# vasil-pashov/sparse_matrix_math

Hardware: AMD Instinct MI355X
Metric: CSR SpMV GB/s (% HBM peak) + BiCGStab iters/sec, 10M rows, 1/2/4/8 GPU (higher is better)
Workload: dtype f32

## Files before the change

include/smm_hip.h:

```cpp
#ifndef SMM_HIP_H
#define SMM_HIP_H

#include <stddef.h>

#ifdef __cplusplus
extern "C" {
#endif

#define SMM_HIP_VERSION_MAJOR 0
#define SMM_HIP_VERSION_MINOR 1

#define SMM_HIP_OK 0
#define SMM_HIP_ERR_INVALID (-1)
#define SMM_HIP_ERR_HIP (-2)
#define SMM_HIP_ERR_NO_DEVICE (-3)
#define SMM_HIP_ERR_PRECOND (-4)
#define SMM_HIP_ERR_NOMEM (-5)
#define SMM_HIP_ERR_COMM (-6)

#define SMM_SOLVER_SUCCESS 0
#define SMM_SOLVER_DIVERGED 1
#define SMM_SOLVER_MAX_ITERATIONS_REACHED 2

#define SMM_OP_ASSIGN 0
// ... 23 lines not shown

typedef struct smm_hip_csr smm_hip_csr;
typedef struct smm_hip_precond smm_hip_precond;
typedef void* smm_hip_stream;

int smm_hip_init(int device);
int smm_hip_shutdown(void);
const char* smm_hip_last_error(void);
int smm_hip_uses_std_fma(void);
int smm_hip_device_info(char* name, size_t name_cap, int* cus, size_t* hbm_bytes);
int smm_hip_stream_synchronize(smm_hip_stream stream);

int smm_hip_debug_fail_next_alloc(size_t min_bytes);
int smm_hip_profile_enable(int on);
int smm_hip_profile_read(double* spmv_ms, long long* spmv_launches, int reset);
int smm_hip_profile_read_waits(double* exposed_ms, long long* pairs, int reset);

int smm_hip_csr_create_f32(int rows, int cols, const int* start, const int* positions, const float* values, smm_hip_csr** out);
int smm_hip_csr_create_f64(int rows, int cols, const int* start, const int* positions, const double* values, smm_hip_csr** out);
int smm_hip_csr_create_dev_f32(int rows, int cols, const int* d_start, const int* d_positions, const float* d_values, smm_hip_csr** out);
int smm_hip_csr_create_dev_f64(int rows, int cols, const int* d_start, const int* d_positions, const double* d_values, smm_hip_csr** out);
int smm_hip_csr_destroy(smm_hip_csr* m);
int smm_hip_csr_info(const smm_hip_csr* m, int* rows, int* cols, int* nnz, int* dtype, int* first_active_start);
int smm_hip_csr_set_kernel(smm_hip_csr* m, int family, int lanes_per_row);
int smm_hip_csr_get_kernel(const smm_hip_csr* m, int* family, int* lanes_per_row);
int smm_hip_csr_tile_info(const smm_hip_csr* m, int* tiles, int* tile_nnz_cap, int* tile_max_rows, int* tile_kernel);
int smm_hip_csr_pattern_info(const smm_hip_csr* m, int* encoding, int* offsets);
int smm_hip_csr_kernel_desc(const smm_hip_csr* m, char* name, int name_cap, long long* bytes_per_launch);
int smm_hip_set_march_min_rows(long long const_diagonals_rows, long long values_read_rows);
int smm_hip_set_cg_lazy_x_min_bytes(long long bytes);
int smm_hip_set_cg_fuse_p(int on);
int smm_hip_csr_pattern_allow_const(smm_hip_csr* m, int allow);
int smm_hip_csr_pattern_slots(smm_hip_csr* m, int mode);
int smm_hip_csr_autotune(smm_hip_csr* m);

#define SMM_UPDATE_SET 0
#define SMM_UPDATE_ADD 1
int smm_hip_csr_scale_f32(smm_hip_csr* m, float alpha, smm_hip_stream stream);
int smm_hip_csr_scale_f64(smm_hip_csr* m, double alpha, smm_hip_stream stream);
int smm_hip_csr_axpy_f32(smm_hip_csr* m, float alpha, const smm_hip_csr* other, smm_hip_stream stream);
int smm_hip_csr_axpy_f64(smm_hip_csr* m, double alpha, const smm_hip_csr* other, smm_hip_stream stream);
int smm_hip_csr_zero_f32(smm_hip_csr* m, smm_hip_stream stream);
int smm_hip_csr_zero_f64(smm_hip_csr* m, smm_hip_stream stream);
int smm_hip_csr_update_entries_f32(smm_hip_csr* m, int n, const int* rows, const int* cols, const float* values, int mode, unsigned char* found);
int smm_hip_csr_update_entries_f64(smm_hip_csr* m, int n, const int* rows, const int* cols, const double* values, int mode, unsigned char* found);
int smm_hip_csr_update_entries_dev_f32(smm_hip_csr* m, int n, const int* d_rows, const int* d_cols, const float* d_values, int mode, unsigned char* d_found,
                                       smm_hip_stream stream);
int smm_hip_csr_update_entries_dev_f64(smm_hip_csr* m, int n, const int* d_rows, const int* d_cols, const double* d_values, int mode, unsigned char* d_found,
                                       smm_hip_stream stream);
int smm_hip_csr_set_values_f32(smm_hip_csr* m, const float* values);
int smm_hip_csr_set_values_f64(smm_hip_csr* m, const double* values);
int smm_hip_csr_set_values_dev_f32(smm_hip_csr* m, const float* d_values, smm_hip_stream stream);
int smm_hip_csr_set_values_dev_f64(smm_hip_csr* m, const double* d_values, smm_hip_stream stream);
int smm_hip_csr_get_values_f32(const smm_hip_csr* m, float* values);
int smm_hip_csr_get_values_f64(const smm_hip_csr* m, double* values);
int smm_hip_csr_values_changed_f32(smm_hip_csr* m, smm_hip_stream stream);
int smm_hip_csr_values_changed_f64(smm_hip_csr* m, smm_hip_stream stream);
int smm_hip_csr_same_pattern(const smm_hip_csr* a, const smm_hip_csr* b, int* same);

int smm_hip_spmv_f32(const smm_hip_csr* m, int op, const float* lhs, const float* x, float* out);
int smm_hip_spmv_f64(const smm_hip_csr* m, int op, const double* lhs, const double* x, double* out);
int smm_hip_spmv_dev_f32(const smm_hip_csr* m, int op, const float* d_lhs, const float* d_x, float* d_out, smm_hip_stream stream);
int smm_hip_spmv_dev_f64(const smm_hip_csr* m, int op, const double* d_lhs, const double* d_x, double* d_out, smm_hip_stream stream);

int smm_hip_dot_f32(int n, const float* a, const float* b, float* result);
int smm_hip_dot_f64(int n, const double* a, const double* b, double* result);
// ... 177 lines not shown
```

sparse_matrix_math_amd/_lib.py:

```python
import ctypes
import os
from ctypes import POINTER, c_char_p, c_double, c_float, c_int, c_longlong, c_size_t, c_ulonglong, c_void_p

_HERE = os.path.dirname(os.path.abspath(__file__))

SMM_HIP_OK = 0
SMM_HIP_ERR_INVALID = -1
SMM_HIP_ERR_HIP = -2
SMM_HIP_ERR_NO_DEVICE = -3
SMM_HIP_ERR_PRECOND = -4
SMM_HIP_ERR_NOMEM = -5
SMM_HIP_ERR_COMM = -6


class SmmHipError(RuntimeError):
    def __init__(self, code, message):
        super().__init__(f"libsmm_hip error {code}: {message}")
        self.code = code


def library_path(fma=False):
    if os.environ.get("SMM_HIP_LIBRARY"):
        return os.environ["SMM_HIP_LIBRARY"]
    name = "libsmm_hip_fma.so" if fma else "libsmm_hip.so"
# ... 46 lines not shown
    "smm_hip_csr_update_entries_dev": (c_int, [_P, c_int, _P, _P, _P, c_int, _P, _P]),
    "smm_hip_csr_set_values": (c_int, [_P, _P]),
    "smm_hip_csr_set_values_dev": (c_int, [_P, _P, _P]),
    "smm_hip_csr_get_values": (c_int, [_P, _P]),
    "smm_hip_csr_values_changed": (c_int, [_P, _P]),
}



_PLAIN = {
    "smm_hip_init": (c_int, [c_int]),
    "smm_hip_shutdown": (c_int, []),
    "smm_hip_last_error": (c_char_p, []),
    "smm_hip_uses_std_fma": (c_int, []),
    "smm_hip_device_info": (c_int, [c_char_p, c_size_t, POINTER(c_int), POINTER(c_size_t)]),
    "smm_hip_stream_synchronize": (c_int, [_P]),
    "smm_hip_debug_fail_next_alloc": (c_int, [c_size_t]),
    "smm_hip_profile_enable": (c_int, [c_int]),
    "smm_hip_profile_read": (c_int, [POINTER(c_double), POINTER(c_longlong), c_int]),
    "smm_hip_profile_read_waits": (c_int, [POINTER(c_double), POINTER(c_longlong), c_int]),
    "smm_hip_csr_destroy": (c_int, [_P]),
    "smm_hip_csr_info": (c_int, [_P, POINTER(c_int), POINTER(c_int), POINTER(c_int), POINTER(c_int), POINTER(c_int)]),
    "smm_hip_csr_set_kernel": (c_int, [_P, c_int, c_int]),
    "smm_hip_csr_get_kernel": (c_int, [_P, POINTER(c_int), POINTER(c_int)]),
    "smm_hip_csr_autotune": (c_int, [_P]),
    "smm_hip_csr_tile_info": (c_int, [_P, POINTER(c_int), POINTER(c_int), POINTER(c_int), POINTER(c_int)]),
    "smm_hip_csr_pattern_info": (c_int, [_P, POINTER(c_int), POINTER(c_int)]),
    "smm_hip_csr_kernel_desc": (c_int, [_P, c_char_p, c_int, POINTER(c_longlong)]),
    "smm_hip_set_march_min_rows": (c_int, [c_longlong, c_longlong]),
    "smm_hip_set_cg_lazy_x_min_bytes": (c_int, [c_longlong]),
    "smm_hip_set_cg_fuse_p": (c_int, [c_int]),
    "smm_hip_csr_pattern_allow_const": (c_int, [_P, c_int]),
    "smm_hip_csr_pattern_slots": (c_int, [_P, c_int]),
    "smm_hip_csr_same_pattern": (c_int, [_P, _P, POINTER(c_int)]),
    "smm_hip_precond_create": (c_int, [_P, c_int, POINTER(_P)]),
    "smm_hip_precond_create_block": (c_int, [_P, c_int, c_int, POINTER(_P)]),
    "smm_hip_precond_create_block_capped": (c_int, [_P, c_int, c_int, c_int, POINTER(_P)]),
    "smm_hip_precond_block_level_cap": (c_int, [_P, POINTER(c_int)]),
    "smm_hip_precond_create_block_ex": (c_int, [_P, c_int, c_int, c_int, c_int, POINTER(_P)]),
    "smm_hip_precond_block_rows": (c_int, [_P, _P, c_size_t, _P]),
    "smm_hip_precond_block_record_bytes": (c_int, [_P, POINTER(c_int), POINTER(c_int), POINTER(c_int)]),
    "smm_hip_precond_block_count": (c_int, [_P, POINTER(c_int)]),
    "smm_hip_precond_block_bounds": (c_int, [_P, _P, c_size_t]),
    "smm_hip_precond_destroy": (c_int, [_P]),
    "smm_hip_precond_set_sweep": (c_int, [_P, c_int]),
    "smm_hip_precond_take_error": (c_int, [_P, _P]),
    "smm_hip_precond_info": (c_int, [_P, POINTER(c_int), POINTER(c_int), POINTER(c_int)]),
    "smm_hip_gen_poisson2d_nnz": (c_longlong, [c_int, c_int]),
    "smm_hip_gen_stencil3d_nnz": (c_longlong, [c_int, c_int, c_int]),
    "smm_hip_gen_banded_nnz": (c_longlong, [c_int, c_int, c_ulonglong, c_int]),
    "smm_hip_gen_banded_row_start": (c_longlong, [c_int, c_int, c_ulonglong, c_int, c_int]),
    "smm_hip_partials_count": (c_int, []),
    "smm_hip_finish_len": (c_int, []),
    "smm_hip_finish_totals_offset": (c_int, []),
    "smm_hip_cg_resident": (c_int, [c_int]),
    "smm_hip_bicgstab_resident": (c_int, [c_int]),
    "smm_hip_bicgstab_ws_destroy": (c_int, [_P]),
    "smm_hip_cg_ws_status": (c_int, [_P, _P, POINTER(c_int)]),
    "smm_hip_bicgstab_ws_bind": (c_int, [_P, _P, _P, _P]),
    "smm_hip_bicgstab_ws_pointers": (c_int, [_P, POINTER(_P), POINTER(_P), POINTER(_P), POINTER(_P), POINTER(_P), POINTER(_P)]),
    "smm_hip_comm_unique_id": (c_int, [_P]),
    "smm_hip_comm_create_rccl": (c_int, [c_int, c_int, _P, POINTER(_P)]),
    "smm_hip_comm_create_host": (c_int, [c_int, c_int, HOST_ALLREDUCE_FN, HOST_SENDRECV_FN, _P, POINTER(_P)]),
    "smm_hip_comm_create_self": (c_int, [POINTER(_P)]),
    "smm_hip_comm_destroy": (c_int, [_P]),
    "smm_hip_comm_info": (c_int, [_P, POINTER(c_int), POINTER(c_int), POINTER(c_int)]),
# ... 86 lines not shown
```

sparse_matrix_math_amd/csrc/smm_internal.h:

```cpp
#pragma once
#include <hip/hip_runtime.h>

#include <cstddef>
#include <cstdint>
#include <cstdio>
#include <atomic>
#include <chrono>
#include <cstdlib>
#include <cstring>
#include <mutex>
#include <string>
#include <type_traits>
#include <vector>

#include "../../include/smm_hip.h"

namespace smm {

void setError(const char* fmt, ...);
int hipFail(hipError_t e, const char* what, const char* file, int line);

#define SMM_HIP_TRY(expr)                                             \
	do {                                                              \
		hipError_t _e = (expr);                                       \
// ... 179 lines not shown
constexpr int SPMV_ADD_DIV = 0x1000;
constexpr int SPMV_OP_ADD_DIV = 4;
constexpr int SPMV_HALF_TILES = 0x2000;
constexpr int SPMV_NO_FULL_ROWS = 0x4000;
constexpr int PARTS_TOTALS = 2 * NPART;
constexpr int PARTS_TICKETS = 16;
constexpr int PARTS_LEN = 2 * NPART + 2 + 2 * (PARTS_TICKETS + 1);
template <typename T>
__host__ __device__ inline unsigned* partsTicket(T* partials) { return reinterpret_cast<unsigned*>(partials + PARTS_TOTALS + 2); }
inline int spmvOutFlags(const smm_hip_csr* m, size_t elemBytes) {
	static const int forced = [] {
		const char* env = getenv("SMM_HIP_NT_OUT");
		return env ? atoi(env) : -1;
	}();
	if (forced >= 0) return forced ? SPMV_NT_OUT : 0;
	return static_cast<double>(m->rows) * static_cast<double>(elemBytes) >= 64.0 * 1024 * 1024 ? SPMV_NT_OUT : 0;
}

int buildRowBlocks(smm_hip_csr* m, int capNnz, int maxRows, hipStream_t s);
int buildTileTable(const smm_hip_csr* m, int capNnz, int maxRows, hipStream_t s, int** blocks, int* nBlocks, int* chunkTiles);
int cutRows(const int* d_start, int rows, long long nnz, int capNnz, int maxRows, hipStream_t s, int2** tiles, int* nTiles, int tilesPerChunk = 0);
int ensureCsrReady(const smm_hip_csr* m, hipStream_t s, bool streamKnown);
int ensurePattern(smm_hip_csr* m, hipStream_t s = nullptr, bool streamKnown = false, bool quiet = false, bool masksOnly = false);
int adoptPatternForSolver(const smm_hip_csr* m, int plannedIterations, hipStream_t s);
void adoptPatternQuietly(const smm_hip_csr* m, hipStream_t s);
int patternLanesFor(const smm_hip_csr* m);
const char* patternKernelDesc(const smm_hip_csr* m, int lanes, long long* bytes);
void planMarch(smm_hip_csr* m);
int refreshResEll(smm_hip_csr* a, hipStream_t s);
bool ensurePatternSlots(smm_hip_csr* m, int lanes, hipStream_t s);
bool patternSlotsChosen(const smm_hip_csr* m, int lanes);
long long patternSlotsBytes(const smm_hip_csr* m);
int refreshPatternSlots(smm_hip_csr* m, hipStream_t s);
int marchBuildMasks32(smm_hip_csr* m, hipStream_t s);
template <typename K>
inline int occupancyCached(std::atomic<long long>& slot, K kernel, int tpb, size_t lds, int fallback) {
	const long long seen = slot.load(std::memory_order_acquire);
	if (seen != 0 && static_cast<size_t>(seen >> 8) == lds) return static_cast<int>(seen & 0xFF);
	int n = 0;
	if (hipOccupancyMaxActiveBlocksPerMultiprocessor(&n, kernel, tpb, lds) != hipSuccess || n < 1) {
		(void)hipGetLastError();
		n = fallback;
	}
	n = n > 255 ? 255 : n;
	slot.store((static_cast<long long>(lds) << 8) | n, std::memory_order_release);
	return n;
}
template <typename K>
inline bool ensureDynamicLds(std::atomic<int>& granted, K kernel, size_t lds) {
	if (lds <= 64 * 1024) return true;
	int have = granted.load(std::memory_order_acquire);
	while (static_cast<size_t>(have) < lds) {
		if (hipFuncSetAttribute(reinterpret_cast<const void*>(kernel), hipFuncAttributeMaxDynamicSharedMemorySize, static_cast<int>(lds)) != hipSuccess) {
			(void)hipGetLastError();
			return false;
		}
		if (granted.compare_exchange_weak(have, static_cast<int>(lds), std::memory_order_acq_rel)) break;
	}
	return true;
}
inline int forcedWgsPerCU() {
	static const int forced = [] {
		const char* env = getenv("SMM_HIP_STREAM_WGS_PER_CU");
		return env ? (atoi(env) > 1 ? atoi(env) : 1) : 0;
	}();
	return forced;
}

bool cgHalfTiles(const smm_hip_csr* m, size_t elemBytes);
long long cgLazyMinBytes();
bool updateNT(long long n, size_t elemBytes, int vectors);
bool masksMarchApplies(const smm_hip_csr* m);
bool constMarchApplies(const smm_hip_csr* m);
template <typename T>
bool launchPatMasksMarch(const smm_hip_csr* m, int op, const T* lhs, const T* divisor, const T* x, T* out, int dotMode, const T* w1, T* partials,
                         const int* doneFlag, hipStream_t s);
template <typename T>
bool launchPatConstMarch(const smm_hip_csr* m, int op, const T* lhs, const T* divisor, const T* x, T* out, int dotMode, const T* w1, T* partials,
                         const int* doneFlag, hipStream_t s);
template <typename T>
void launchPatSlots(const smm_hip_csr* m, int lanes, int op, const T* lhs, const T* divisor, const T* x, T* out, int dotMode, const T* w1, T* partials,
                    const int* doneFlag, hipStream_t s);
template <typename T>
int launchSpmvPattern(const smm_hip_csr* m, int lanes, int op, const T* lhs, const T* divisor, const T* x, T* out, int dotMode, const T* w1, T* partials,
                      const int* doneFlag, hipStream_t s);
void chooseSpmvConfig(smm_hip_csr* m);
template <typename T>
int launchSpmvSplit(const smm_hip_csr* aLoc, const smm_hip_csr* aRem, int op, const T* lhs, const T* divisor, const T* own, const T* ext, T* out, int dotMode,
                    const T* w1, T* partials, const int* doneFlag, int extraFlags, const unsigned long long* landed, unsigned long long seq, unsigned long long* err,
                    long long ticks, hipStream_t s, const struct P2PSlotArgs* slots = nullptr, int sumsLdsMax = 16384, unsigned long long* waited = nullptr);
void launchSplitSignal(unsigned long long* landed, unsigned long long seq, hipStream_t s);
void preloadSplitUnit();
template <typename T>
struct CgFuseBook {
	const int* pad = nullptr;
	T* rrPing = nullptr;
	T* res = nullptr;
	int *iters = nullptr, *done = nullptr, *status = nullptr, *flushIter = nullptr;
};
template <typename T>
struct CgFuseArgs {
	const T* r;
	T* pNew;
	CgFuseBook<T> bk;
	const T* partsC;
	T eps;
	int par, iter;
	const T* totalsC = nullptr;
	int extraFlags = 0;
};
bool constMarchFusable(const smm_hip_csr* m, size_t elemBytes);
template <typename T>
bool launchConstMarchFusedP(const smm_hip_csr* m, const T* pOld, T* Ap, T* partials, const int* doneFlag, const CgFuseArgs<T>& f, hipStream_t s);

template <typename T>
// ... 100 lines not shown
```

sparse_matrix_math_amd/csrc/smm_spmv_pattern.hip:

```cpp
#include <algorithm>
#include <cmath>

#include <rocprim/device/device_radix_sort.hpp>

#include "smm_device.h"
#include "smm_internal.h"
#include "smm_pattern_dev.h"

namespace smm {

__global__ __launch_bounds__(TPB) void patBuildMasks(int rows, const int* __restrict__ meta, const int* __restrict__ offs, const int* __restrict__ start,
                                                     const int* __restrict__ positions, unsigned long long* __restrict__ masks,
                                                     int* __restrict__ flags, const void* __restrict__ values, int elemBytes,
                                                     const unsigned long long* __restrict__ cvalBits) {
	if (meta[1] != 0) return;
	const int k = meta[0];
	if (values != nullptr && k > 32) values = nullptr;
	int* mismatch = flags;
	__shared__ int sOff[MAXOFF];
	__shared__ unsigned long long sCval[MAXOFF];
	const bool checkConst = values != nullptr && flags[1] == 0;
	if (checkConst && threadIdx.x < k) sCval[threadIdx.x] = cvalBits[threadIdx.x];
	bool varies = false;
	__shared__ int sRow[TPB / WAVE][WAVE + 1];
// ... 1465 lines not shown
		return "spmvDictKernel";
	}
	if (L == 1 && m->pat_const && !m->pat_const_off) {
		static const bool marchOn = [] {
			const char* env = getenv("SMM_HIP_CONST_MARCH");
			return env ? atoi(env) != 0 : true;
		}();
		const bool march = marchOn && constMarchApplies(m);
		const bool bytesMasks = march && !m->march_clusters && m->d_pat_masks8 && m->pat_k - m->march_lo - m->march_hi == 5;
		*bytes = rows * (bytesMasks ? 1 : march ? 4 : 8) + vectors;
		return march ? (m->march_clusters ? "spmvPatternConstMarch3Kernel" : "spmvPatternConstMarchKernel") : "spmvPatternConstKernel";
	}
	*bytes = nnz * s + rows * 8 + startBytes + vectors;
	if (L == 1 && masksMarchApplies(m)) {
		static const bool masksMarchOn = [] {
			const char* env = getenv("SMM_HIP_MASKS_MARCH");
			return env ? atoi(env) != 0 : true;
		}();
		if (masksMarchOn) {
			*bytes = nnz * s + rows + (rows / 64 + 1) * 4 + vectors;
			return "spmvPatternMasksMarchKernel";
		}
	}
	if (L == 1) {
		static const int waveEnv = [] {
			const char* env = getenv("SMM_HIP_PATTERN_WAVE");
			return env ? atoi(env) : -1;
		}();
		if (waveEnv != 0 && m->pat_k <= 16) return "spmvPatternWaveKernel";
	}
	if ((L == 2 || L == 4) && patUseTile(L)) {
		if (patternSlotsChosen(m, L)) {
			*bytes = patternSlotsBytes(m);
			return "spmvPatternSlotsKernel";
		}
		return "spmvPatternTileKernel";
	}
	return "spmvPatternKernel";
}

static bool patNeedsTiles(const smm_hip_csr* m, int L) {
	if (L != 1 || m->pat_encoding != 0) return true;
	if (m->pat_const && !m->pat_const_off) return false;
	static const int waveEnv = [] {
		const char* env = getenv("SMM_HIP_PATTERN_WAVE");
		return env ? atoi(env) : -1;
	}();
	return !(waveEnv != 0 && m->pat_k <= 16);
}

static int buildPatternTiles(smm_hip_csr* m, int capNnz, int maxRows, hipStream_t s) {
	int* blocks = nullptr;
	int n = 0, chunk = 0;
	SMM_TRY(buildTileTable(m, capNnz, maxRows, s, &blocks, &n, &chunk));
	devFree(m->d_pat_rowblocks);
	m->d_pat_rowblocks = blocks;
	m->pat_n_rowblocks = n;
	m->pat_nnz_cap = capNnz;
	m->pat_max_rows = maxRows;
	m->pat_chunk_tiles = chunk;
	return SMM_HIP_OK;
}

template <typename T>
int launchSpmvPattern(const smm_hip_csr* m, int lanes, int op, const T* lhs, const T* divisor, const T* x, T* out, int dotMode, const T* w1, T* partials,
                      const int* doneFlag, hipStream_t s) {
	auto* mm = const_cast<smm_hip_csr*>(m);
// ... 52 lines not shown
```

sparse_matrix_math_amd/csrc/smm_spmv_slots.hip:

```cpp
#include <algorithm>

#include <rocprim/device/device_scan.hpp>

#include "smm_pattern_dev.h"

namespace smm {

constexpr int SLOT_WAVES = TPB / WAVE;

__global__ __launch_bounds__(TPB) void slotsCountKernel(int rows, int nWaves, const unsigned long long* __restrict__ masks, long long* __restrict__ counts,
                                                        int* __restrict__ uniformWaves) {
	const int lane = threadIdx.x & (WAVE - 1);
	int mine = 0;
	for (int w = (blockIdx.x * TPB + threadIdx.x) / WAVE; w < nWaves; w += gridDim.x * SLOT_WAVES) {
		const int row = w * WAVE + lane;
		const unsigned long long mm = row < rows ? masks[row] : ~0ULL;
		const unsigned long long lead = patUniform64(mm);
		const bool uniform = lead != 0ULL && __builtin_amdgcn_ballot_w64(!(row < rows && mm == lead)) == 0ULL;
		if (lane == 0) {
			counts[w] = uniform ? static_cast<long long>(__builtin_popcountll(lead)) * WAVE : 0;
			mine += uniform;
		}
	}
	if (lane == 0 && mine) atomicAdd(uniformWaves, mine);
}

__global__ __launch_bounds__(TPB) void slotsMarkKernel(int nWaves, const long long* __restrict__ counts, long long* __restrict__ base) {
	for (int w = blockIdx.x * TPB + threadIdx.x; w < nWaves; w += gridDim.x * TPB) {
		if (counts[w] == 0) base[w] = -1;
	}
}

template <typename T>
__global__ __launch_bounds__(TPB) void slotsFillKernel(int nWaves, const long long* __restrict__ base, const unsigned long long* __restrict__ masks,
                                                       const int* __restrict__ start, const T* __restrict__ values, T* __restrict__ slots) {
	const int lane = threadIdx.x & (WAVE - 1);
	for (int w = (blockIdx.x * TPB + threadIdx.x) / WAVE; w < nWaves; w += gridDim.x * SLOT_WAVES) {
		const long long b = base[w];
		if (b < 0) continue;
		const int row = w * WAVE + lane;
		const int len = __builtin_popcountll(masks[w * WAVE]);
// ... 57 lines not shown
				}
			}
			dot = part[0];
#pragma unroll
			for (int q = 1; q < L; ++q) dot += part[q];
		} else if (row < rows) {
			dot = patRowDirect<T, L>(start[row], start[row + 1], values, positions, x);
		}
		if (row < rows) {
			const T o = patApplyOp(op, lhs, divisor, row, dot);
			storeOut(out + row, o, ntOut);
			if (dotMode == 2) acc0 += o * o;
			if (dotMode) acc1 += o * w1[row];
		}
	}
	if (dotMode) {
		if (dotMode == 2) {
			const T s0 = blockSum256(acc0, red);
			if (t == 0) partials[blockIdx.x] = s0;
		}
		const T s1 = blockSum256(acc1, red);
		if (t == 0) partials[(dotMode == 2 ? NPART : 0) + blockIdx.x] = s1;
		for (int i = gridDim.x + blockIdx.x * TPB + t; i < NPART; i += gridDim.x * TPB) {
			partials[i] = T(0);
			if (dotMode == 2) partials[NPART + i] = T(0);
		}
		if (opFlags & SPMV_FINISH) lastBlockSums<T>(partials, NPART, dotMode == 2 ? 2 : 1, partials + PARTS_TOTALS, partsTicket(partials));
	}
}

static int slotsEnvMode() {
	static const int mode = [] {
		const char* env = getenv("SMM_HIP_PATTERN_SLOTS");
		return env ? (atoi(env) != 0 ? 1 : 0) : -1;
	}();
	return mode;
}

static int slotsMode(const smm_hip_csr* m) { return m->pat_slots_mode >= 0 ? m->pat_slots_mode : slotsEnvMode(); }

static bool slotsApplies(const smm_hip_csr* m, int lanes) {
	if (lanes != 2 && lanes != 4) return false;
	if (m->pat_encoding != 0 || (m->pat_const && !m->pat_const_off)) return false;
	static const bool fullRows = [] {
		const char* env = getenv("SMM_HIP_FULL_ROWS");
		const char* variant = getenv("SMM_HIP_PATTERN_VARIANT");
		return !(env && atoi(env) == 0) && !(variant && atoi(variant) == 0);
	}();
	return fullRows;
}

static bool slotsWanted(const smm_hip_csr* m, int lanes, bool* forced) {
	const int mode = slotsMode(m);
	*forced = mode == 1;
	if (mode == 0 || !slotsApplies(m, lanes)) return false;
	return mode == 1 || mode == 2 || !m->kernelForced;
}

static bool slotsUniformEnough(const smm_hip_csr* m) {
	return static_cast<long long>(m->pat_slots_uniform) * 100 >= static_cast<long long>(m->pat_slots_waves) * 99;
}

bool patternSlotsChosen(const smm_hip_csr* m, int lanes) {
	bool forced = false;
	if (!slotsWanted(m, lanes, &forced) || m->pat_slots_state != 1 || !m->d_pat_slots) return false;
	return forced || slotsUniformEnough(m);
}

template <typename T>
static int slotsFill(smm_hip_csr* m, hipStream_t s) {
	const int nWaves = m->pat_slots_waves;
	const int grid = std::max(1, std::min(4096, (nWaves + SLOT_WAVES - 1) / SLOT_WAVES));
	slotsFillKernel<T><<<grid, TPB, 0, s>>>(nWaves, m->d_pat_slot_base, m->d_pat_masks, m->d_start, static_cast<const T*>(m->d_values),
	                                         static_cast<T*>(m->d_pat_slots));
	SMM_HIP_TRY(hipGetLastError());
	return SMM_HIP_OK;
}

template <typename T>
static int slotsBuild(smm_hip_csr* m, bool forced, hipStream_t s) {
	SetupTrace trace("pattern: slots copy");
	const int nWaves = (m->rows + WAVE - 1) / WAVE;
	DevBuf<long long> counts, base;
	DevBuf<int> uniform;
	DevBuf<unsigned char> temp;
	SMM_TRY(counts.alloc(nWaves));
	SMM_TRY(base.alloc(static_cast<size_t>(nWaves) + 1));
	SMM_TRY(uniform.alloc(1));
	SMM_HIP_TRY(hipMemsetAsync(uniform.p, 0, sizeof(int), s));
	SMM_HIP_TRY(hipMemsetAsync(base.p, 0, sizeof(long long), s));
	const int grid = std::max(1, std::min(4096, (nWaves + SLOT_WAVES - 1) / SLOT_WAVES));
	slotsCountKernel<<<grid, TPB, 0, s>>>(m->rows, nWaves, m->d_pat_masks, counts.p, uniform.p);
	SMM_HIP_TRY(hipGetLastError());
	size_t tempBytes = 0;
	SMM_HIP_TRY(rocprim::inclusive_scan(nullptr, tempBytes, counts.p, base.p + 1, static_cast<size_t>(nWaves), rocprim::plus<long long>(), s));
	SMM_TRY(temp.alloc(tempBytes ? tempBytes : 1));
	SMM_HIP_TRY(rocprim::inclusive_scan(temp.p, tempBytes, counts.p, base.p + 1, static_cast<size_t>(nWaves), rocprim::plus<long long>(), s));
	slotsMarkKernel<<<std::max(1, std::min(4096, (nWaves + TPB - 1) / TPB)), TPB, 0, s>>>(nWaves, counts.p, base.p);
	SMM_HIP_TRY(hipGetLastError());
// ... 63 lines not shown
	const int g = (p + nb - 1) / nb;
	return g <= 8 ? 8 : g <= 13 ? 13 : 16;
}

template <typename T, int L, int G>
static void launchSlotsG(const smm_hip_csr* m, int op, const T* lhs, const T* divisor, const T* x, T* out, int dotMode, const T* w1, T* partials,
                         const int* doneFlag, hipStream_t s) {
	static std::atomic<long long> occ{0};
	const int perCU = occupancyCached(occ, spmvPatternSlotsKernel<T, L, G>, TPB, 0, 4);
	const int cus = (op & SPMV_LEAVE_ROOM) ? std::max(8, numCUs() - 8) : numCUs();
	const int nWaves = m->pat_slots_waves;
	const int grid = std::max(1, std::min(std::min((nWaves + SLOT_WAVES - 1) / SLOT_WAVES, cus * perCU), NPART));
	const int nGroups = std::min(8, grid);
	const int chunkWaves = (nWaves + nGroups - 1) / nGroups;
	spmvPatternSlotsKernel<T, L, G><<<grid, TPB, 0, s>>>(m->rows, nWaves, chunkWaves, m->d_pat_off, m->d_pat_slot_base, m->d_pat_masks,
	                                                    static_cast<const T*>(m->d_pat_slots), m->d_start, m->d_positions, static_cast<const T*>(m->d_values),
	                                                    (op & ~SPMV_LEAVE_ROOM) | spmvOutFlags(m, sizeof(T)), lhs, divisor, x, out, dotMode, w1, partials,
	                                                    doneFlag);
}

template <typename T, int L>
static void launchSlotsL(const smm_hip_csr* m, int op, const T* lhs, const T* divisor, const T* x, T* out, int dotMode, const T* w1, T* partials,
                         const int* doneFlag, hipStream_t s) {
	switch (slotsBatch(m, L)) {
	case 8: launchSlotsG<T, L, 8>(m, op, lhs, divisor, x, out, dotMode, w1, partials, doneFlag, s); break;
	case 13: launchSlotsG<T, L, 13>(m, op, lhs, divisor, x, out, dotMode, w1, partials, doneFlag, s); break;
	default: launchSlotsG<T, L, 16>(m, op, lhs, divisor, x, out, dotMode, w1, partials, doneFlag, s); break;
	}
}

template <typename T>
void launchPatSlots(const smm_hip_csr* m, int lanes, int op, const T* lhs, const T* divisor, const T* x, T* out, int dotMode, const T* w1, T* partials,
                    const int* doneFlag, hipStream_t s) {
	if (lanes == 2) {
		launchSlotsL<T, 2>(m, op, lhs, divisor, x, out, dotMode, w1, partials, doneFlag, s);
	} else {
		launchSlotsL<T, 4>(m, op, lhs, divisor, x, out, dotMode, w1, partials, doneFlag, s);
	}
}

template void launchPatSlots<float>(const smm_hip_csr*, int, int, const float*, const float*, const float*, float*, int, const float*, float*, const int*,
                                    hipStream_t);
template void launchPatSlots<double>(const smm_hip_csr*, int, int, const double*, const double*, const double*, double*, int, const double*, double*,
                                     const int*, hipStream_t);

}

extern "C" int smm_hip_csr_pattern_slots(smm_hip_csr* m, int mode) {
	if (!m || mode < -1 || mode > 2) {
		smm::setError("csr_pattern_slots: null matrix or a mode other than -1, 0, 1, 2");
		return SMM_HIP_ERR_INVALID;
	}
	std::lock_guard<std::mutex> lock(m->tileMutex);
	m->pat_slots_mode = mode;
	if (mode == 1 && m->pat_slots_state < 0) m->pat_slots_state = 0;
	return SMM_HIP_OK;
}
```

sparse_matrix_math_amd/host.py:

```python
import ctypes
import enum

import numpy as np

from . import _lib
from ._lib import check


class SolverStatus(enum.IntEnum):
    SUCCESS = 0
    DIVERGED = 1
    MAX_ITERATIONS_REACHED = 2


class SolverPreconditioner(enum.IntEnum):
    NONE = 0
    JACOBI = 1
    ILU0 = 2
    SYMMETRIC_GAUS_SEIDEL = 3
    IC0 = 4
    BLOCK_ILU0 = 5
    BLOCK_SGS = 6


# ... 48 lines not shown

def partials_count():
    return _lib.load().smm_hip_partials_count()


def finish_len():
    return _lib.load().smm_hip_finish_len()


def finish_totals_offset():
    return _lib.load().smm_hip_finish_totals_offset()


def uses_std_fma():
    return bool(_lib.load().smm_hip_uses_std_fma())


def synchronize(stream=None):
    check(_lib.load().smm_hip_stream_synchronize(_dptr(stream)))


def profile_enable(on=True):
    check(_lib.load().smm_hip_profile_enable(1 if on else 0))


def profile_read(reset=True):
    ms, n = ctypes.c_double(), ctypes.c_longlong()
    check(_lib.load().smm_hip_profile_read(ctypes.byref(ms), ctypes.byref(n), 1 if reset else 0))
    return ms.value, n.value


def set_march_min_rows(const_diagonals_rows=-1, values_read_rows=-1):
    check(_lib.load().smm_hip_set_march_min_rows(int(const_diagonals_rows), int(values_read_rows)))


def profile_read_waits(reset=True):
    ms, n = ctypes.c_double(), ctypes.c_longlong()
    check(_lib.load().smm_hip_profile_read_waits(ctypes.byref(ms), ctypes.byref(n), 1 if reset else 0))
    return ms.value, n.value


class Preconditioner:

    def __init__(self, matrix, kind, block_rows=None, level_cap=None, partition=None):
        self.matrix = matrix
        self.kind = SolverPreconditioner(kind)
        self._h = ctypes.c_void_p()
        if block_rows is None and level_cap is None and partition is None:
            check(_lib.load().smm_hip_precond_create(matrix._h, int(kind), ctypes.byref(self._h)))
        elif level_cap is None and partition is None:
            check(_lib.load().smm_hip_precond_create_block(matrix._h, int(kind), int(block_rows), ctypes.byref(self._h)))
        else:
            check(_lib.load().smm_hip_precond_create_block_ex(matrix._h, int(kind), int(block_rows or 0), -1 if level_cap is None else int(level_cap),
                                                               int(partition or 0), ctypes.byref(self._h)))

    def block_record_bytes(self):
        v = [ctypes.c_int() for _ in range(3)]
        check(_lib.load().smm_hip_precond_block_record_bytes(self._h, *[ctypes.byref(c) for c in v]))
        return tuple(c.value for c in v)

    def block_rows(self):
        n = self.matrix.rows
        order = np.zeros(n, dtype=np.int32)
        brick = (ctypes.c_int * 3)()
        check(_lib.load().smm_hip_precond_block_rows(self._h, order.ctypes.data_as(ctypes.c_void_p), n, ctypes.cast(brick, ctypes.c_void_p)))
        return order, tuple(brick)
# ... 363 lines not shown
```

Baseline: 893.5.

## Add row-sweep pattern SpMV kernel that keeps multiple wave-rows open for x reuse

Adds a new pattern-slots SpMV kernel in which each wave processes several consecutive 64-row groups at once. Waves are partitioned into per-XCD chunks so that x accesses across diagonals stay within a narrow sweeping window and hit in cache, instead of each diagonal front streaming x separately. A host heuristic compares the diagonal gaps against the swept block span to decide when to use it, for f32 only. This adds register pressure from R accumulators and more template instantiations, and the heuristic may pick it on matrices where it does not help.

```diff
diff --git a/include/smm_hip.h b/include/smm_hip.h
--- a/include/smm_hip.h
+++ b/include/smm_hip.h
@@ -79,6 +79,7 @@
 int smm_hip_set_cg_fuse_p(int on);
 int smm_hip_csr_pattern_allow_const(smm_hip_csr* m, int allow);
 int smm_hip_csr_pattern_slots(smm_hip_csr* m, int mode);
+int smm_hip_set_pattern_sweep_rows(int rows_open);
 int smm_hip_csr_autotune(smm_hip_csr* m);
 
 #define SMM_UPDATE_SET 0
diff --git a/sparse_matrix_math_amd/_lib.py b/sparse_matrix_math_amd/_lib.py
--- a/sparse_matrix_math_amd/_lib.py
+++ b/sparse_matrix_math_amd/_lib.py
@@ -102,6 +102,7 @@
     "smm_hip_set_cg_fuse_p": (c_int, [c_int]),
     "smm_hip_csr_pattern_allow_const": (c_int, [_P, c_int]),
     "smm_hip_csr_pattern_slots": (c_int, [_P, c_int]),
+    "smm_hip_set_pattern_sweep_rows": (c_int, [c_int]),
     "smm_hip_csr_same_pattern": (c_int, [_P, _P, POINTER(c_int)]),
     "smm_hip_precond_create": (c_int, [_P, c_int, POINTER(_P)]),
     "smm_hip_precond_create_block": (c_int, [_P, c_int, c_int, POINTER(_P)]),
diff --git a/sparse_matrix_math_amd/csrc/smm_internal.h b/sparse_matrix_math_amd/csrc/smm_internal.h
--- a/sparse_matrix_math_amd/csrc/smm_internal.h
+++ b/sparse_matrix_math_amd/csrc/smm_internal.h
@@ -235,6 +235,8 @@
 bool patternSlotsChosen(const smm_hip_csr* m, int lanes);
 long long patternSlotsBytes(const smm_hip_csr* m);
 int refreshPatternSlots(smm_hip_csr* m, hipStream_t s);
+int patternSweepRows(const smm_hip_csr* m, int lanes);
+int patternSweepGroupWaves(const smm_hip_csr* m, int lanes, int rowsOpen);
 int marchBuildMasks32(smm_hip_csr* m, hipStream_t s);
 template <typename K>
 inline int occupancyCached(std::atomic<long long>& slot, K kernel, int tpb, size_t lds, int fallback) {
@@ -284,6 +286,9 @@
 template <typename T>
 void launchPatSlots(const smm_hip_csr* m, int lanes, int op, const T* lhs, const T* divisor, const T* x, T* out, int dotMode, const T* w1, T* partials,
                     const int* doneFlag, hipStream_t s);
+template <typename T>
+void launchPatSweep(const smm_hip_csr* m, int lanes, int rowsOpen, int op, const T* lhs, const T* divisor, const T* x, T* out, int dotMode, const T* w1,
+                    T* partials, const int* doneFlag, hipStream_t s);
 template <typename T>
 int launchSpmvPattern(const smm_hip_csr* m, int lanes, int op, const T* lhs, const T* divisor, const T* x, T* out, int dotMode, const T* w1, T* partials,
                       const int* doneFlag, hipStream_t s);
diff --git a/sparse_matrix_math_amd/csrc/smm_spmv_pattern.hip b/sparse_matrix_math_amd/csrc/smm_spmv_pattern.hip
--- a/sparse_matrix_math_amd/csrc/smm_spmv_pattern.hip
+++ b/sparse_matrix_math_amd/csrc/smm_spmv_pattern.hip
@@ -1521,7 +1521,7 @@
 	if ((L == 2 || L == 4) && patUseTile(L)) {
 		if (patternSlotsChosen(m, L)) {
 			*bytes = patternSlotsBytes(m);
-			return "spmvPatternSlotsKernel";
+			return patternSweepRows(m, L) ? "spmvPatternSweepKernel" : "spmvPatternSlotsKernel";
 		}
 		return "spmvPatternTileKernel";
 	}
diff --git a/sparse_matrix_math_amd/csrc/smm_spmv_slots.hip b/sparse_matrix_math_amd/csrc/smm_spmv_slots.hip
--- a/sparse_matrix_math_amd/csrc/smm_spmv_slots.hip
+++ b/sparse_matrix_math_amd/csrc/smm_spmv_slots.hip
@@ -7,6 +7,11 @@
 namespace smm {
 
 constexpr int SLOT_WAVES = TPB / WAVE;
+
+constexpr int SWEEP_ROWS_DEFAULT = 16;
+constexpr int SWEEP_MIN_BLOCKS = 3;
+constexpr long long SWEEP_FRONT_REACH = 16384;
+constexpr double SWEEP_MIN_RATIO = 1.5;
 
 __global__ __launch_bounds__(TPB) void slotsCountKernel(int rows, int nWaves, const unsigned long long* __restrict__ masks, long long* __restrict__ counts,
                                                         int* __restrict__ uniformWaves) {
@@ -130,7 +135,7 @@
 static int slotsEnvMode() {
 	static const int mode = [] {
 		const char* env = getenv("SMM_HIP_PATTERN_SLOTS");
-		return env ? (atoi(env) != 0 ? 1 : 0) : -1;
+		return env ? (atoi(env) == 3 ? 3 : atoi(env) != 0 ? 1 : 0) : -1;
 	}();
 	return mode;
 }
@@ -150,9 +155,9 @@
 
 static bool slotsWanted(const smm_hip_csr* m, int lanes, bool* forced) {
 	const int mode = slotsMode(m);
-	*forced = mode == 1;
+	*forced = mode == 1 || mode == 3;
 	if (mode == 0 || !slotsApplies(m, lanes)) return false;
-	return mode == 1 || mode == 2 || !m->kernelForced;
+	return mode >= 1 || !m->kernelForced;
 }
 
 static bool slotsUniformEnough(const smm_hip_csr* m) {
@@ -163,6 +168,40 @@
 	bool forced = false;
 	if (!slotsWanted(m, lanes, &forced) || m->pat_slots_state != 1 || !m->d_pat_slots) return false;
 	return forced || slotsUniformEnough(m);
+}
+
+static std::atomic<int> g_sweepRows{0};
+
+static int sweepRowsOpen() {
+	if (const int forced = g_sweepRows.load(std::memory_order_relaxed)) return forced;
+	static const int env = [] {
+		const char* e = getenv("SMM_HIP_PATTERN_SWEEP_ROWS");
+		const int r = e ? atoi(e) : 0;
+		return r == 8 || r == 16 || r == 32 ? r : 0;
+	}();
+	return env ? env : SWEEP_ROWS_DEFAULT;
+}
+
+static bool sweepSpanWins(const smm_hip_csr* m, long long blockRows) {
+	const std::vector<int>& offs = m->pat_offs_host;
+	double front = 1.0, sweep = 1.0;
+	for (size_t i = 1; i < offs.size(); ++i) {
+		const long long gap = static_cast<long long>(offs[i]) - offs[i - 1];
+		if (gap > SWEEP_FRONT_REACH) front += 1.0;
+		sweep += static_cast<double>(std::min(gap, blockRows)) / static_cast<double>(blockRows);
+	}
+	return sweep * SWEEP_MIN_RATIO <= front;
+}
+
+int patternSweepRows(const smm_hip_csr* m, int lanes) {
+	const int mode = slotsMode(m);
+	const int r = sweepRowsOpen();
+	if (mode == 3) return r;
+	if (mode == 1 || mode == 0) return 0;
+	if (m->dtype != SMM_DTYPE_F32) return 0;
+	const long long groupWaves = patternSweepGroupWaves(m, lanes, r);
+	if (m->pat_slots_waves / 8 < SWEEP_MIN_BLOCKS * groupWaves) return 0;
+	return sweepSpanWins(m, groupWaves * WAVE) ? r : 0;
 }
 
 template <typename T>
@@ -292,6 +331,10 @@
 template <typename T>
 void launchPatSlots(const smm_hip_csr* m, int lanes, int op, const T* lhs, const T* divisor, const T* x, T* out, int dotMode, const T* w1, T* partials,
                     const int* doneFlag, hipStream_t s) {
+	if (const int rowsOpen = patternSweepRows(m, lanes)) {
+		launchPatSweep<T>(m, lanes, rowsOpen, op, lhs, divisor, x, out, dotMode, w1, partials, doneFlag, s);
+		return;
+	}
 	if (lanes == 2) {
 		launchSlotsL<T, 2>(m, op, lhs, divisor, x, out, dotMode, w1, partials, doneFlag, s);
 	} else {
@@ -307,12 +350,21 @@
 }
 
 extern "C" int smm_hip_csr_pattern_slots(smm_hip_csr* m, int mode) {
-	if (!m || mode < -1 || mode > 2) {
-		smm::setError("csr_pattern_slots: null matrix or a mode other than -1, 0, 1, 2");
+	if (!m || mode < -1 || mode > 3) {
+		smm::setError("csr_pattern_slots: null matrix or a mode other than -1, 0, 1, 2, 3");
 		return SMM_HIP_ERR_INVALID;
 	}
 	std::lock_guard<std::mutex> lock(m->tileMutex);
 	m->pat_slots_mode = mode;
-	if (mode == 1 && m->pat_slots_state < 0) m->pat_slots_state = 0;
+	if ((mode == 1 || mode == 3) && m->pat_slots_state < 0) m->pat_slots_state = 0;
 	return SMM_HIP_OK;
 }
+
+extern "C" int smm_hip_set_pattern_sweep_rows(int rows_open) {
+	if (rows_open != 0 && rows_open != 8 && rows_open != 16 && rows_open != 32) {
+		smm::setError("set_pattern_sweep_rows: 8, 16, 32, or 0 for the default");
+		return SMM_HIP_ERR_INVALID;
+	}
+	smm::g_sweepRows.store(rows_open, std::memory_order_relaxed);
+	return SMM_HIP_OK;
+}
diff --git a/sparse_matrix_math_amd/csrc/smm_spmv_sweep.hip b/sparse_matrix_math_amd/csrc/smm_spmv_sweep.hip
--- /dev/null
+++ b/sparse_matrix_math_amd/csrc/smm_spmv_sweep.hip
@@ -0,0 +1,238 @@
+#include <algorithm>
+
+#include "smm_pattern_dev.h"
+
+namespace smm {
+
+constexpr int SWEEP_WAVES = TPB / WAVE;
+
+__device__ __forceinline__ unsigned long long sweepLane64(unsigned hi, unsigned lo, int j) {
+	const unsigned h = __builtin_amdgcn_readlane(hi, j), l = __builtin_amdgcn_readlane(lo, j);
+	return (static_cast<unsigned long long>(h) << 32) | l;
+}
+
+template <typename T, int L, int R>
+__global__ __launch_bounds__(TPB) void spmvPatternSweepKernel(int rows, int nWaves, int chunkWaves, const int* __restrict__ offs,
+                                                              const long long* __restrict__ base, const unsigned long long* __restrict__ masks,
+                                                              const T* __restrict__ slots, const int* __restrict__ start, const int* __restrict__ positions,
+                                                              const T* __restrict__ values, int opFlags, const T* lhs, const T* __restrict__ divisor,
+                                                              const T* __restrict__ x, T* out, int dotMode, const T* __restrict__ w1,
+                                                              T* __restrict__ partials, const int* __restrict__ doneFlag) {
+	static_assert(L == 2 || L == 4, "pieces per row");
+	static_assert(R >= 1 && R <= 32, "rows of waves held open");
+	constexpr int JB = R < 16 ? R : 16;
+	static_assert(R % JB == 0, "whole batches");
+	__shared__ T red[4];
+	if (doneFlag && *doneFlag) return;
+	const int op = opFlags & 0xFF;
+	const bool ntOut = (opFlags & SPMV_NT_OUT) != 0;
+	const int t = threadIdx.x;
+	const unsigned lane = t & (WAVE - 1);
+	const int wave = __builtin_amdgcn_readfirstlane(t >> 6);
+	const int nGroups = min(8, static_cast<int>(gridDim.x));
+	const int xcdGroup = blockIdx.x % nGroups;
+	const int groupWgs = (static_cast<int>(gridDim.x) - xcdGroup + nGroups - 1) / nGroups;
+	const int hwWaves = groupWgs * SWEEP_WAVES;
+	const int hw = static_cast<int>(blockIdx.x / nGroups) * SWEEP_WAVES + wave;
+	const int gBegin = min(nWaves, xcdGroup * chunkWaves), gEnd = min(nWaves, (xcdGroup + 1) * chunkWaves);
+	const int gWaves = gEnd - gBegin;
+	const int nSuper = (gWaves + hwWaves * R - 1) / (hwWaves * R);
+	const int superWaves = nSuper ? (gWaves + nSuper - 1) / nSuper : 0;
+	const int per = (superWaves + hwWaves - 1) / hwWaves;
+	T acc0 = T(0), acc1 = T(0);
+	for (int sb = 0; sb < nSuper; ++sb) {
+		const int sBegin = gBegin + sb * superWaves, sEnd = min(gEnd, sBegin + superWaves);
+		const int first = sBegin + hw * per;
+		const int cnt = max(0, min(per, sEnd - first));
+		if (cnt == 0) continue;
+		long long bj = -1;
+		unsigned long long mj = 0ULL;
+		if (static_cast<int>(lane) < cnt) {
+			bj = base[first + static_cast<int>(lane)];
+			if (bj >= 0) mj = masks[static_cast<long long>(first + static_cast<int>(lane)) * WAVE];
+		}
+		const unsigned long long have = __builtin_amdgcn_ballot_w64(bj >= 0);
+		for (unsigned long long rest = ~have & ((1ULL << cnt) - 1ULL); rest; rest &= rest - 1ULL) {
+			const int row = (first + __builtin_ctzll(rest)) * WAVE + static_cast<int>(lane);
+			if (row < rows) {
+				const T dot = patRowDirect<T, L>(start[row], start[row + 1], values, positions, x);
+				const T o = patApplyOp(op, lhs, divisor, row, dot);
+				storeOut(out + row, o, ntOut);
+				if (dotMode == 2) acc0 += o * o;
+				if (dotMode) acc1 += o * w1[row];
+			}
+		}
+		if (have == 0ULL) continue;
+		const int ref = __builtin_ctzll(have);
+		const long long bRef = static_cast<long long>(sweepLane64(static_cast<unsigned>(bj >> 32), static_cast<unsigned>(bj), ref));
+		const unsigned vLo = static_cast<unsigned>(mj), vHi = static_cast<unsigned>(mj >> 32);
+		const int vRel = bj >= 0 ? static_cast<int>(bj - bRef) : 0;
+		unsigned long long todo = 0ULL;
+		for (unsigned long long h = have; h; h &= h - 1ULL) {
+			const int j = __builtin_ctzll(h);
+			todo |= sweepLane64(vHi, vLo, j);
+		}
+		const T* const sv = slots + bRef;
+		const int row0 = first * WAVE;
+		T acc[R], sum[R];
+#pragma unroll
+		for (int j = 0; j < R; ++j) acc[j] = sum[j] = T(0);
+		const unsigned long long lead0 = sweepLane64(vHi, vLo, 0);
+		if (have == (1ULL << cnt) - 1ULL && __builtin_amdgcn_ballot_w64(static_cast<int>(lane) < cnt && mj != lead0) == 0ULL) {
+			const int len = __builtin_popcountll(lead0);
+			const int pl = (len + L - 1) / L;
+			const unsigned stride = static_cast<unsigned>(len) * WAVE;
+			int done = 0;
+			for (todo = lead0; todo; todo &= todo - 1ULL) {
+				const T* const ve = sv + static_cast<unsigned>(done) * WAVE;
+				const T* const xe = x + (row0 + offs[__builtin_ctzll(todo)]);
+				T vv[R], xv[R];
+#pragma unroll
+				for (int j = 0; j < R; ++j) {
+					if (j < cnt) {
+						vv[j] = __builtin_nontemporal_load(ve + j * stride + lane);
+						xv[j] = xe[j * WAVE + lane];
+					}
+				}
+#pragma unroll
+				for (int j = 0; j < R; ++j) {
+					if (j < cnt) acc[j] = smmFma(vv[j], xv[j], acc[j]);
+				}
+				++done;
+				if (done == len || done == pl || (L == 4 && (done == 2 * pl || done == 3 * pl))) {
+#pragma unroll
+					for (int j = 0; j < R; ++j) {
+						sum[j] = done <= pl ? acc[j] : sum[j] + acc[j];
+						acc[j] = T(0);
+					}
+				}
+			}
+		}
+		for (; todo; todo &= todo - 1ULL) {
+			const int e = __builtin_ctzll(todo);
+			const unsigned long long below = (1ULL << e) - 1ULL;
+			const int off = offs[e];
+#pragma unroll
+			for (int jb = 0; jb < R; jb += JB) {
+				T vv[JB], xv[JB];
+#pragma unroll
+				for (int u = 0; u < JB; ++u) {
+					const int j = jb + u;
+					const unsigned long long lead = sweepLane64(vHi, vLo, j);
+					if ((lead >> e) & 1ULL) {
+						const int entry = __builtin_popcountll(lead & below);
+						const int rel = __builtin_amdgcn_readlane(vRel, j) + entry * WAVE;
+						vv[u] = __builtin_nontemporal_load(sv + rel + lane);
+						xv[u] = x[static_cast<long long>(row0 + j * WAVE + off) + lane];
+					}
+				}
+#pragma unroll
+				for (int u = 0; u < JB; ++u) {
+					const int j = jb + u;
+					const unsigned long long lead = sweepLane64(vHi, vLo, j);
+					if ((lead >> e) & 1ULL) {
+						acc[j] = smmFma(vv[u], xv[u], acc[j]);
+						const int done = __builtin_popcountll(lead & below) + 1;
+						const int len = __builtin_popcountll(lead);
+						const int pl = (len + L - 1) / L;
+						const bool closes = done == len || done == pl || (L == 4 && (done == 2 * pl || done == 3 * pl));
+						if (closes) {
+							sum[j] = done <= pl ? acc[j] : sum[j] + acc[j];
+							acc[j] = T(0);
+						}
+					}
+				}
+			}
+		}
+#pragma unroll
+		for (int j = 0; j < R; ++j) {
+			if ((have >> j) & 1ULL) {
+				const int row = row0 + j * WAVE + static_cast<int>(lane);
+				const T o = patApplyOp(op, lhs, divisor, row, sum[j]);
+				storeOut(out + row, o, ntOut);
+				if (dotMode == 2) acc0 += o * o;
+				if (dotMode) acc1 += o * w1[row];
+			}
+		}
+	}
+	if (dotMode) {
+		if (dotMode == 2) {
+			const T s0 = blockSum256(acc0, red);
+			if (t == 0) partials[blockIdx.x] = s0;
+		}
+		const T s1 = blockSum256(acc1, red);
+		if (t == 0) partials[(dotMode == 2 ? NPART : 0) + blockIdx.x] = s1;
+		for (int i = gridDim.x + blockIdx.x * TPB + t; i < NPART; i += gridDim.x * TPB) {
+			partials[i] = T(0);
+			if (dotMode == 2) partials[NPART + i] = T(0);
+		}
+		if (opFlags & SPMV_FINISH) lastBlockSums<T>(partials, NPART, dotMode == 2 ? 2 : 1, partials + PARTS_TOTALS, partsTicket(partials));
+	}
+}
+
+static int sweepWgsPerCU() {
+	static const int n = [] {
+		const char* env = getenv("SMM_HIP_PATTERN_SWEEP_WGS");
+		return env ? std::max(1, std::min(8, atoi(env))) : 3;
+	}();
+	return n;
+}
+
+template <typename T, int L, int R>
+static int sweepWgsOf() {
+	static std::atomic<long long> occ{0};
+	return std::max(1, std::min(sweepWgsPerCU(), occupancyCached(occ, spmvPatternSweepKernel<T, L, R>, TPB, 0, 1)));
+}
+
+template <typename T, int L>
+static int sweepWgsOfR(int rowsOpen) {
+	return rowsOpen == 8 ? sweepWgsOf<T, L, 8>() : rowsOpen == 16 ? sweepWgsOf<T, L, 16>() : sweepWgsOf<T, L, 32>();
+}
+
+int patternSweepGroupWaves(const smm_hip_csr* m, int lanes, int rowsOpen) {
+	const int wgs = m->dtype == SMM_DTYPE_F32 ? (lanes == 2 ? sweepWgsOfR<float, 2>(rowsOpen) : sweepWgsOfR<float, 4>(rowsOpen))
+	                                          : (lanes == 2 ? sweepWgsOfR<double, 2>(rowsOpen) : sweepWgsOfR<double, 4>(rowsOpen));
+	return ((numCUs() * wgs + 7) / 8) * SWEEP_WAVES * rowsOpen;
+}
+
+template <typename T, int L, int R>
+static void launchSweepR(const smm_hip_csr* m, int op, const T* lhs, const T* divisor, const T* x, T* out, int dotMode, const T* w1, T* partials,
+                         const int* doneFlag, hipStream_t s) {
+	const int perCU = sweepWgsOf<T, L, R>();
+	const int cus = (op & SPMV_LEAVE_ROOM) ? std::max(8, numCUs() - 8) : numCUs();
+	const int nWaves = m->pat_slots_waves;
+	const int grid = std::max(1, std::min(std::min((nWaves + SWEEP_WAVES - 1) / SWEEP_WAVES, cus * perCU), NPART));
+	const int nGroups = std::min(8, grid);
+	const int chunkWaves = (nWaves + nGroups - 1) / nGroups;
+	spmvPatternSweepKernel<T, L, R><<<grid, TPB, 0, s>>>(m->rows, nWaves, chunkWaves, m->d_pat_off, m->d_pat_slot_base, m->d_pat_masks,
+	                                                    static_cast<const T*>(m->d_pat_slots), m->d_start, m->d_positions, static_cast<const T*>(m->d_values),
+	                                                    (op & ~SPMV_LEAVE_ROOM) | spmvOutFlags(m, sizeof(T)), lhs, divisor, x, out, dotMode, w1, partials,
+	                                                    doneFlag);
+}
+
+template <typename T, int L>
+static void launchSweepL(const smm_hip_csr* m, int rowsOpen, int op, const T* lhs, const T* divisor, const T* x, T* out, int dotMode, const T* w1,
+                         T* partials, const int* doneFlag, hipStream_t s) {
+	switch (rowsOpen) {
+	case 8: launchSweepR<T, L, 8>(m, op, lhs, divisor, x, out, dotMode, w1, partials, doneFlag, s); break;
+	case 16: launchSweepR<T, L, 16>(m, op, lhs, divisor, x, out, dotMode, w1, partials, doneFlag, s); break;
+	default: launchSweepR<T, L, 32>(m, op, lhs, divisor, x, out, dotMode, w1, partials, doneFlag, s); break;
+	}
+}
+
+template <typename T>
+void launchPatSweep(const smm_hip_csr* m, int lanes, int rowsOpen, int op, const T* lhs, const T* divisor, const T* x, T* out, int dotMode, const T* w1,
+                    T* partials, const int* doneFlag, hipStream_t s) {
+	if (lanes == 2) {
+		launchSweepL<T, 2>(m, rowsOpen, op, lhs, divisor, x, out, dotMode, w1, partials, doneFlag, s);
+	} else {
+		launchSweepL<T, 4>(m, rowsOpen, op, lhs, divisor, x, out, dotMode, w1, partials, doneFlag, s);
+	}
+}
+
+template void launchPatSweep<float>(const smm_hip_csr*, int, int, int, const float*, const float*, const float*, float*, int, const float*, float*,
+                                    const int*, hipStream_t);
+template void launchPatSweep<double>(const smm_hip_csr*, int, int, int, const double*, const double*, const double*, double*, int, const double*, double*,
+                                     const int*, hipStream_t);
+
+}
diff --git a/sparse_matrix_math_amd/host.py b/sparse_matrix_math_amd/host.py
--- a/sparse_matrix_math_amd/host.py
+++ b/sparse_matrix_math_amd/host.py
@@ -104,6 +104,10 @@
 
 def set_march_min_rows(const_diagonals_rows=-1, values_read_rows=-1):
     check(_lib.load().smm_hip_set_march_min_rows(int(const_diagonals_rows), int(values_read_rows)))
+
+
+def set_pattern_sweep_rows(rows_open=0):
+    check(_lib.load().smm_hip_set_pattern_sweep_rows(int(rows_open)))
 
 
 def profile_read_waits(reset=True):
```

Measured after the change: 958.9, median of 6. 7.3% higher.
